# jianwang-mpi/SceneEgo

Hardware: NVIDIA B200
Metric: frames/s VoxelNetDepth volumetric stage (higher is better)
Workload: dtype bf16

## Files before the change

### sceneego_b200/build.py

```python
import concurrent.futures
import hashlib
import os
import subprocess
import sys

HERE = os.path.dirname(os.path.abspath(__file__))
CSRC = os.path.join(HERE, "csrc")
LIB = os.path.join(HERE, "libsceneego_b200.so")
LIB_F16 = os.path.join(HERE, "libsceneego_b200_f16.so")
HASH_FILE = LIB + ".srchash"
OBJ_DIR = os.path.join(HERE, "build")
SOURCES = ["geometry.cu", "softargmax.cu", "v2v.cu", "stem.cu", "stem_march.cu", "tail.cu", "march.cu", "eval.cu", "handoff.cu", "feature_conv.cu"]
NVCC_FLAGS = ["-gencode", "arch=compute_100a,code=sm_100a", "-O3", "-lineinfo", "-std=c++17",
              "-Xcompiler", "-fPIC", "-Xptxas", "-v"]


def _sources():
    return [s for s in SOURCES if os.path.exists(os.path.join(CSRC, s))]


def source_hash() -> str:
    h = hashlib.sha256()
    deps = sorted(os.path.join(CSRC, f) for f in os.listdir(CSRC) if f.endswith((".cu", ".cuh", ".h")))
    deps.append(os.path.join(HERE, "..", "include", "sceneego_b200.h"))
    for d in deps:
        h.update(os.path.basename(d).encode())
        h.update(open(d, "rb").read())
    h.update(" ".join(NVCC_FLAGS + _sources()).encode())
    return h.hexdigest()


def recorded_hash() -> str:
    try:
        return open(HASH_FILE).read().strip()
    except OSError:
        return ""


def _stale() -> bool:
    return not (os.path.exists(LIB) and os.path.exists(LIB_F16)) or recorded_hash() != source_hash()


VARIANTS = [("bf16", LIB, []), ("f16", LIB_F16, ["-DSCENEEGO_ACT_F16"])]


def build(force: bool = False, verbose: bool = False) -> str:
    if not force and not _stale():
        return LIB
    nvcc = os.environ.get("NVCC", "/usr/local/cuda/bin/nvcc")
    os.makedirs(OBJ_DIR, exist_ok=True)
    want = source_hash()

    def compile_one(job):
        tag, src, extra = job
        obj = os.path.join(OBJ_DIR, src.replace(".cu", f".{tag}.o"))
        r = subprocess.run([nvcc] + NVCC_FLAGS + extra + ["-c", os.path.join(CSRC, src), "-o", obj], capture_output=True, text=True)
        return tag, src, obj, r

    jobs = [(tag, src, extra) for tag, _, extra in VARIANTS for src in _sources()]
    jobs.sort(key=lambda j: -os.path.getsize(os.path.join(CSRC, j[1])))
    objs = {tag: [] for tag, _, _ in VARIANTS}
    failed = False
    with concurrent.futures.ThreadPoolExecutor(max_workers=min(8, os.cpu_count() or 1)) as ex:
        for tag, src, obj, r in ex.map(compile_one, jobs):
            if verbose or r.returncode != 0:
                sys.stderr.write(f"---- {src} [{tag}]\n{r.stdout}{r.stderr}")
            failed |= r.returncode != 0
            objs[tag].append(obj)
    if failed:
        raise RuntimeError("nvcc failed building libsceneego_b200")
    for tag, lib, _ in VARIANTS:
        r = subprocess.run([nvcc, "--shared", "-gencode", "arch=compute_100a,code=sm_100a", "-o", lib] + objs[tag],
                           capture_output=True, text=True)
        if verbose or r.returncode != 0:
            sys.stderr.write(r.stdout + r.stderr)
        if r.returncode != 0:
            raise RuntimeError(f"nvcc failed linking {os.path.basename(lib)}")
    with open(HASH_FILE, "w") as f:
        f.write(want + "\n")
    return LIB


if __name__ == "__main__":
    print(build(force="--force" in sys.argv, verbose="-q" not in sys.argv))
```

### sceneego_b200/csrc/common.cuh

```cuda
#pragma once
#include <cuda_runtime.h>
#include <cuda_bf16.h>
#include <cuda_fp16.h>
#include <stdint.h>
#include <stdio.h>
#include "../../include/sceneego_b200.h"

namespace sceneego {

#ifdef SCENEEGO_ACT_F16
constexpr int kActDtype = 1;
constexpr uint32_t kIdescAB = 0u;
#define SE_MMA_SYNC_AB ".f16.f16"
__device__ __forceinline__ uint32_t act_pack2(float lo, float hi) {
  uint32_t r;
  asm("cvt.rn.satfinite.f16x2.f32 %0, %1, %2;" : "=r"(r) : "f"(hi), "f"(lo));
  return r;
}
__device__ __forceinline__ uint32_t act_pack2_relu(float lo, float hi) {
  uint32_t r;
  asm("cvt.rn.relu.satfinite.f16x2.f32 %0, %1, %2;" : "=r"(r) : "f"(hi), "f"(lo));
  return r;
}
__device__ __forceinline__ float2 act_unpack2(uint32_t u) { return __half22float2(*reinterpret_cast<const __half2*>(&u)); }
__device__ __forceinline__ __nv_bfloat16 act_from_float(float v) {
  const uint32_t r = act_pack2(v, 0.f);
  const uint16_t lo = (uint16_t)(r & 0xFFFFu);
  return *reinterpret_cast<const __nv_bfloat16*>(&lo);
}
__device__ __forceinline__ float act_to_float(__nv_bfloat16 v) { return __half2float(*reinterpret_cast<const __half*>(&v)); }
#else
constexpr int kActDtype = 0;
constexpr uint32_t kIdescAB = (1u << 7) | (1u << 10);
#define SE_MMA_SYNC_AB ".bf16.bf16"
__device__ __forceinline__ uint32_t act_pack2(float lo, float hi) {
  const __nv_bfloat162 h = __floats2bfloat162_rn(lo, hi);
  return *reinterpret_cast<const uint32_t*>(&h);
}
__device__ __forceinline__ uint32_t act_pack2_relu(float lo, float hi) {
  uint32_t r;
  asm("cvt.rn.relu.bf16x2.f32 %0, %1, %2;" : "=r"(r) : "f"(hi), "f"(lo));
  return r;
}
__device__ __forceinline__ float2 act_unpack2(uint32_t u) { return __bfloat1622float2(*reinterpret_cast<const __nv_bfloat162*>(&u)); }
__device__ __forceinline__ __nv_bfloat16 act_from_float(float v) { return __float2bfloat16(v); }
__device__ __forceinline__ float act_to_float(__nv_bfloat16 v) { return __bfloat162float(v); }
#endif

void set_error(const char* fmt, ...);
int ensure_max_dynamic_smem(const void* kernel, int bytes);

#define SE_REQUIRE(cond, ...)                      \
  do {                                             \
    if (!(cond)) {                                 \
      ::sceneego::set_error(__VA_ARGS__);          \
      return SCENEEGO_E_INVALID;                   \
    }                                              \
  } while (0)

#define SE_CUDA_LAUNCH_CHECK(what)                                              \
  do {                                                                          \
    cudaError_t e__ = cudaGetLastError();                                       \
    if (e__ != cudaSuccess) {                                                   \
      ::sceneego::set_error("%s: %s", what, cudaGetErrorString(e__));           \
      return SCENEEGO_E_CUDA;                                                   \
    }                                                                           \
  } while (0)

struct CalibDev {
  double cx, cy;
  double c2w[7];
  double w2c[11];
  int width, height;
};

inline CalibDev to_dev(const sceneego_calib_t* c) {
  CalibDev d;
  d.cx = c->cx; d.cy = c->cy;
  for (int i = 0; i < 7; ++i) d.c2w[i] = c->c2w[i];
  for (int i = 0; i < 11; ++i) d.w2c[i] = c->w2c[i];
  d.width = c->width; d.height = c->height;
  return d;
}

__host__ __device__ inline int64_t vol_pos(const sceneego_vol_layout_t& L, int b, int x, int y, int z) {
  return (int64_t)b * L.frame_pitch + L.guard + (int64_t)x * L.pitch_x + (int64_t)y * L.pitch_y + z;
}

__device__ __forceinline__ float voxel_coord(float lo, float step, int i) {
  return __fadd_rn(lo, __fmul_rn(step, (float)i));
}

__host__ __device__ inline int64_t vol_cell(const sceneego_vol_layout_t& L, int b, int x, int y, int z, int g, int C8) {
  if (L.s2d) {
    const int par = ((x & 1) << 2) | ((y & 1) << 1) | (z & 1);
    return (int64_t)(par * C8 + g) * L.plane_stride + vol_pos(L, b, x >> 1, y >> 1, z >> 1);
  }
  return (int64_t)g * L.plane_stride + vol_pos(L, b, x, y, z);
}
__host__ __device__ inline int64_t vol_scene_elem(const sceneego_vol_layout_t& L, int b, int x, int y, int z, int C8) {
  if (L.s2d) {
    const int par = ((x & 1) << 2) | ((y & 1) << 1) | (z & 1);
    return ((int64_t)(8 * C8) * L.plane_stride + vol_pos(L, b, x >> 1, y >> 1, z >> 1)) * 8 + par;
  }
  return ((int64_t)C8 * L.plane_stride + vol_pos(L, b, x, y, z)) * 8;
}

constexpr int kNumSMs = 148;

int launch_stem_s2d(const sceneego_v2v_op_t& op, void* const* d_buffers, const void* d_blob, int batch, int op_index,
                    bool simt, cudaStream_t st);
int launch_feature_conv1x1_simt(const float* d_feat, const float* d_weight, const float* d_bias, float* d_out, int batch,
                                int cin, int cout, int h, int w, cudaStream_t st);
int launch_stem_march(const sceneego_v2v_op_t& op, void* const* d_buffers, const void* d_blob, int batch, int op_index,
                      bool simt, cudaStream_t st);
int launch_tail_mlp(const sceneego_v2v_op_t& op, void* const* d_buffers, const void* d_blob, int batch, int op_index,
                    bool simt, cudaStream_t st);
int launch_conv_march(const sceneego_v2v_op_t& op, void* const* d_buffers, const void* d_blob, int batch, int op_index,
                      cudaStream_t st);

}
```

### sceneego_b200/csrc/v2v.cu

```cuda
#include "tc_common.cuh"
#include <stdarg.h>
#include <stdlib.h>
#include <string.h>
#include <math.h>
#include <mutex>

namespace sceneego {


struct ConvParams {
  const __nv_bfloat16* src;
  __nv_bfloat16* dst;
  const __nv_bfloat16* res;
  float* dst_f32;
  const __nv_bfloat16* w;
  const float* bias;
  sceneego_vol_layout_t ls, ld;
  int batch;
  int k, r, cin_planes, ksteps, N, cout_real, flags;
  int xs, n0, n_dx, n_xg, items_per_plane;
  FastDiv fd_frame, fd_px, fd_py;
  int deconv, par0;
  int taps_dx;
  int mma_n;
// ... 611 lines not shown
  }
  *reinterpret_cast<uint4*>(dst + ((int64_t)g * ld.plane_stride + vol_pos(ld, b, x, y, z)) * 8) = pack8(m);
}

__global__ void __launch_bounds__(128) deconv2_kernel(const __grid_constant__ ConvParams p) {
  const int So = p.ld.side;
  const int n = blockIdx.x * blockDim.x + threadIdx.x;
  const int go = blockIdx.y, b = blockIdx.z;
  if (n >= So * So * So) return;
  const int z = n % So, y = (n / So) % So, x = n / (So * So);
  const int tap = ((x & 1) * 2 + (y & 1)) * 2 + (z & 1);
  const int64_t qs = vol_pos(p.ls, b, x >> 1, y >> 1, z >> 1);
  float acc[8];
#pragma unroll
  for (int j = 0; j < 8; ++j) acc[j] = 0.f;
  for (int g = 0; g < p.cin_planes; ++g) {
    float a[8];
    unpack8(*reinterpret_cast<const uint4*>(p.src + ((int64_t)g * p.ls.plane_stride + qs) * 8), a);
    int npar = 256 / p.N;
    if (npar > 8) npar = 8;
    const uint4* wrow = reinterpret_cast<const uint4*>(p.w) +
                        ((size_t)(tap / npar) * p.cin_planes + g) * ((size_t)npar * p.N) + (size_t)(tap % npar) * p.N + go * 8;
#pragma unroll
    for (int j = 0; j < 8; ++j) {
      float wv[8];
      unpack8(__ldg(wrow + j), wv);
#pragma unroll
      for (int i = 0; i < 8; ++i) acc[j] = fmaf(a[i], wv[i], acc[j]);
    }
  }
  const int64_t cell = (int64_t)go * p.ld.plane_stride + vol_pos(p.ld, b, x, y, z);
  float rr[8];
  if (p.flags & SCENEEGO_F_ADD_AFTER) unpack8(*reinterpret_cast<const uint4*>(p.res + cell * 8), rr);
#pragma unroll
  for (int j = 0; j < 8; ++j) {
    float t = acc[j] + p.bias[go * 8 + j];
    if (p.flags & SCENEEGO_F_RELU) t = fmaxf(t, 0.f);
    if (p.flags & SCENEEGO_F_ADD_AFTER) t += rr[j];
    acc[j] = t;
  }
  *reinterpret_cast<uint4*>(p.dst + cell * 8) = pack8(acc);
}

static thread_local char g_err[512] = "";
int ensure_max_dynamic_smem(const void* kernel, int bytes) {
  struct Entry { int dev; const void* fn; int bytes; };
  static Entry seen[512];
  static int n_seen = 0;
  static std::mutex mu;
  int dev = 0;
  cudaError_t e = cudaGetDevice(&dev);
  if (e != cudaSuccess) { set_error("cudaGetDevice: %s", cudaGetErrorString(e)); return SCENEEGO_E_CUDA; }
  std::lock_guard<std::mutex> lock(mu);
  for (int i = 0; i < n_seen; ++i)
    if (seen[i].dev == dev && seen[i].fn == kernel && seen[i].bytes >= bytes) return SCENEEGO_OK;
  e = cudaFuncSetAttribute(kernel, cudaFuncAttributeMaxDynamicSharedMemorySize, bytes);
  if (e != cudaSuccess) { set_error("cudaFuncSetAttribute(MaxDynamicSharedMemorySize): %s", cudaGetErrorString(e)); return SCENEEGO_E_CUDA; }
  if (n_seen < 512) seen[n_seen++] = Entry{dev, kernel, bytes};
  return SCENEEGO_OK;
}

void set_error(const char* fmt, ...) {
  va_list ap;
  va_start(ap, fmt);
  vsnprintf(g_err, sizeof(g_err), fmt, ap);
  va_end(ap);
}
static thread_local int g_launches = 0;

static bool try_plan(ConvParams& p, int tiles, int want_stages) {
  const int taps_dx = p.taps_dx;
  const int L = tiles * 128;
  const int WL = L + 2 * p.r * (p.ls.pitch_y + 1);
  const uint32_t win_bytes = (uint32_t)WL * 16u;
  const uint32_t stage = win_bytes * p.cin_planes;
  const uint32_t fixed = 1024;
  if ((uint64_t)stage * want_stages + fixed > kMaxSmem) return false;
  const uint32_t used = stage * want_stages + fixed;
  const uint32_t room = kMaxSmem - used;
  int wct = taps_dx, wrows = 0;
  if (p.k == 3 && !p.deconv && 3u * 9u * p.tap_bytes <= room) { wct = 9; wrows = 3; }
  else if (p.k == 3 && !p.deconv && 2u * 3u * p.tap_bytes <= room) { wct = 3; wrows = 1; }
  else {
    while (wct > 1 && (uint32_t)wct * p.tap_bytes > 24576u) {
      int nx = wct - 1;
      while (nx > 1 && taps_dx % nx) --nx;
      wct = nx;
    }
  }
  { const char* e = getenv("SCENEEGO_WCHUNK"); if (e && atoi(e) > 0 && taps_dx % atoi(e) == 0) { wct = atoi(e); wrows = (p.k == 3 && !p.deconv && wct % 3 == 0) ? wct / 3 : 0; if (wrows == 2) wrows = 0; } }
  const uint32_t wchunk = (uint32_t)wct * p.tap_bytes;
  if (2ull * wchunk > room) return false;
  int slots = (int)(room / wchunk);
  if (slots > MAX_WSLOTS) slots = MAX_WSLOTS;
  if (slots > 4 && wchunk > 8192) slots = 4;
  { const char* e = getenv("SCENEEGO_WSLOTS"); if (e && atoi(e) >= 2 && atoi(e) <= MAX_WSLOTS && (uint64_t)used + (uint64_t)atoi(e) * wchunk <= kMaxSmem) slots = atoi(e); }
  p.wrows = wrows;
  p.tiles = tiles; p.L = L; p.WL = WL;
  p.win_bytes = win_bytes; p.win_stages = want_stages;
  p.wchunk_taps = wct; p.wchunks_per_dx = taps_dx / wct; p.wchunk_bytes = wchunk; p.w_slots = slots;
  p.off_win = 0;
  p.off_w = stage * want_stages;
  p.off_bias = p.off_w + wchunk * slots;
  p.off_bar = p.off_bias + 512;
  p.half_cols = (uint32_t)(tiles * p.N);
  uint32_t cols = 32;
  while (cols < 2 * p.half_cols) cols <<= 1;
  p.tmem_cols = cols;
  return true;
}

static int plan_conv(ConvParams& p, int64_t n_pos) {
  p.tap_bytes = (uint32_t)p.cin_planes * (p.mma_n / p.cg) * 16u;
  int max_tiles = 256 / p.N;
  if (max_tiles > 8) max_tiles = 8;
  if (p.xs == 1 && p.cg == 1) {
    auto items_of = [&](int t) { return (n_pos + (int64_t)t * 128 - 1) / ((int64_t)t * 128); };
    if (items_of(max_tiles) < 4 * kNumSMs) {
      int best = max_tiles;
      int64_t best_cost = ((items_of(max_tiles) + kNumSMs - 1) / kNumSMs) * max_tiles;
      for (int t = max_tiles >> 1; t >= 1; t >>= 1) {
        const int64_t cost = ((items_of(t) + kNumSMs - 1) / kNumSMs) * t;
        if (cost < best_cost) { best_cost = cost; best = t; }
      }
      max_tiles = best;
    }
  }
  const char* et = getenv("SCENEEGO_TILES");
  const char* es = getenv("SCENEEGO_STAGES");
  if (et || es) {
    const int tiles = et ? atoi(et) : max_tiles;
    const int stages = es ? atoi(es) : 2;
    if (tiles >= 1 && tiles <= max_tiles && stages >= 1 && stages <= MAX_STAGES && try_plan(p, tiles, stages))
      return (int)(p.off_bar + 512);
  }
  const int first_stages = p.k == 1 ? 4 : (p.cg == 2 || p.cin_planes <= 2) ? 3 : 2;
  for (int tiles = max_tiles; tiles >= 1; tiles >>= 1)
    for (int stages = first_stages; stages >= 2; --stages)
      if (try_plan(p, tiles, stages)) return (int)(p.off_bar + 512);
  return -1;
}

}

using namespace sceneego;

extern "C" int sceneego_abi_version(void) { return SCENEEGO_ABI_VERSION; }
extern "C" int sceneego_act_dtype(void) { return kActDtype; }
extern "C" const char* sceneego_last_error(void) { return g_err; }
extern "C" int sceneego_v2v_last_launch_count(void) { return g_launches; }

extern "C" int sceneego_v2v_pack_conv(const float* h_weight, const float* h_bias, const float* h_gamma,
                                      const float* h_beta, const float* h_mean, const float* h_var, double eps,
                                      int cout, int cin, int ksize, int transposed, int cout_pad, int cin_pad,
                                      int xstack, int n_split, uint16_t* h_w_out, float* h_b_out) {
  SE_REQUIRE(h_weight && h_w_out && h_b_out, "pack_conv: null argument");
  SE_REQUIRE(cout_pad >= cout && cin_pad >= cin && cout_pad % 8 == 0 && cin_pad % 8 == 0, "pack_conv: bad padding");
  SE_REQUIRE(xstack >= 1 && (xstack == 1 || !transposed), "pack_conv: bad xstack");
  SE_REQUIRE(n_split == 1 || (n_split == 2 && !transposed && (xstack * cout_pad) % 32 == 0), "pack_conv: bad n_split");
  const int taps = ksize * ksize * ksize;
  const int kk = ksize * ksize;
  const int n_stk = xstack * cout_pad;
  const int n_dx = ksize + xstack - 1;
  memset(h_w_out, 0, (size_t)n_dx * kk * cin_pad * n_stk * sizeof(uint16_t));
  for (int co = 0; co < cout_pad; ++co) {
    double scale = 1.0, shift = 0.0;
    if (co < cout) {
      if (h_gamma) {
        scale = (double)h_gamma[co] / sqrt((double)h_var[co] + eps);
        shift = (double)h_beta[co] - (double)h_mean[co] * scale;
      }
      h_b_out[co] = (float)((h_bias ? (double)h_bias[co] : 0.0) * scale + shift);
    } else {
      h_b_out[co] = 0.f;
    }
    if (co >= cout) continue;
    for (int ci = 0; ci < cin; ++ci)
      for (int t = 0; t < taps; ++t) {
        const size_t src = transposed ? (((size_t)ci * cout + co) * taps + t) : (((size_t)co * cin + ci) * taps + t);
        const uint16_t wv = f2bf((float)((double)h_weight[src] * scale));
        const int dx = t / kk, rest = t % kk;
        if (transposed) {
          int npar = 256 / cout_pad;
          if (npar > 8) npar = 8;
          const size_t grp = (size_t)t / npar, nrow = (size_t)(t % npar) * cout_pad + co;
          h_w_out[((grp * (cin_pad / 8) + ci / 8) * ((size_t)npar * cout_pad) + nrow) * 8 + (ci & 7)] = wv;
          continue;
        }
        for (int sft = 0; sft < xstack; ++sft) {
          const size_t tp = (size_t)(dx + sft) * kk + rest;
          const size_t col = (size_t)sft * cout_pad + co;
          const size_t nh = (size_t)n_stk / n_split, hf = col / nh;
          const size_t half_elems = (size_t)n_dx * kk * cin_pad * nh;
          const size_t dst = hf * half_elems + ((tp * (cin_pad / 8) + ci / 8) * nh + (col - hf * nh)) * 8 + (ci & 7);
          h_w_out[dst] = wv;
        }
      }
  }
  return SCENEEGO_OK;
}

static int launch_conv_tc(ConvParams& p, int batch, int op_index, cudaStream_t st) {
  p.n0_shift = -1;
  for (int k = 3; k < 10; ++k) if ((1 << k) == p.n0) p.n0_shift = k;
  const int64_t n_pos = (int64_t)batch * p.ls.frame_pitch;
  SE_REQUIRE(n_pos + 4096 < (1ll << 31) && (n_pos + 4096) * (int64_t)p.ls.frame_pitch < (1ll << 48),
             "v2v_run: op %d: batch * frame_pitch too large for one launch (use a smaller chunk)", op_index);
  p.fd_frame = make_fastdiv((uint32_t)p.ls.frame_pitch);
  p.fd_px = make_fastdiv((uint32_t)p.ls.pitch_x);
  p.fd_py = make_fastdiv((uint32_t)p.ls.pitch_y);
  const int smem = plan_conv(p, n_pos);
  SE_REQUIRE(smem > 0, "v2v_run: op %d does not fit shared memory", op_index);
  if (p.xs == 1) {
    p.n_items = (int)((n_pos + p.L - 1) / p.L);
  } else {
    p.items_per_plane = (p.ls.pitch_x + p.L - 1) / p.L;
    p.n_xg = (p.ls.side + p.xs - 1) / p.xs;
    p.n_items = batch * p.n_xg * p.items_per_plane;
  }
  int grid = p.n_items < kNumSMs ? p.n_items : kNumSMs;
  conv_tc_fn fn = nullptr;
  p.w_main_bytes = (uint32_t)(p.n_dx * p.taps_dx) * p.tap_bytes;
  p.w_half_bytes = p.w_main_bytes + (uint32_t)p.n_dx2 * (p.tap_bytes / 2);
  if (p.cg == 2) {
    const int groups = (p.n_items + 1) / 2;
    grid = 2 * (groups < kNumSMs / 2 ? groups : kNumSMs / 2);
    fn = pick_conv_tc_pair(p.ksteps, p.tiles, p.xs, p.wrows);
  } else {
    fn = pick_conv_tc(p.ksteps, p.tiles, p.xs, p.wrows);
    if (fn == nullptr && p.wrows != 0) { p.wrows = 0; fn = pick_conv_tc(p.ksteps, p.tiles, p.xs, 0); }
  }
  SE_REQUIRE(fn != nullptr, "v2v_run: op %d: no conv_tc instantiation for ksteps=%d tiles=%d xs=%d wrows=%d cta_pair=%d", op_index,
             p.ksteps, p.tiles, p.xs, p.wrows, p.cg);
  if (int rc = ensure_max_dynamic_smem((const void*)fn, (int)kMaxSmem)) return rc;
  if (p.cg == 2) {
    cudaLaunchConfig_t cfg;
    memset(&cfg, 0, sizeof(cfg));
    cfg.gridDim = dim3((unsigned)grid); cfg.blockDim = dim3((unsigned)conv_threads(p.tiles));
    cfg.dynamicSmemBytes = (size_t)smem; cfg.stream = st;
    cudaLaunchAttribute attr;
    attr.id = cudaLaunchAttributeClusterDimension;
    attr.val.clusterDim.x = 2; attr.val.clusterDim.y = 1; attr.val.clusterDim.z = 1;
    cfg.attrs = &attr; cfg.numAttrs = 1;
    cudaError_t e = cudaLaunchKernelEx(&cfg, fn, p);
    if (e != cudaSuccess) { set_error("conv_tc (CTA pair): %s", cudaGetErrorString(e)); return SCENEEGO_E_CUDA; }
  } else {
    fn<<<grid, conv_threads(p.tiles), (size_t)smem, st>>>(p);
  }
  SE_CUDA_LAUNCH_CHECK("conv_tc");
  ++g_launches;
  return SCENEEGO_OK;
}

static int v2v_run_impl(const sceneego_v2v_op_t* ops, int n_ops, void* const* d_buffers, const void* d_blob,
                        int batch, void* stream, cudaEvent_t* ev) {
  SE_REQUIRE(ops && d_buffers && d_blob && n_ops > 0 && batch > 0, "v2v_run: bad argument");
  cudaStream_t st = (cudaStream_t)stream;
  const char* force_simt = getenv("SCENEEGO_FORCE_SIMT");
  g_launches = 0;
  for (int i = 0; i < n_ops; ++i) {
    if (ev) cudaEventRecord(ev[i], st);
    const sceneego_v2v_op_t& op = ops[i];
    ConvParams p;
    memset(&p, 0, sizeof(p));
    p.src = (const __nv_bfloat16*)d_buffers[op.src];
    p.dst = (__nv_bfloat16*)d_buffers[op.dst];
    p.dst_f32 = (float*)d_buffers[op.dst];
    p.res = op.res >= 0 ? (const __nv_bfloat16*)d_buffers[op.res] : nullptr;
    p.ls = op.lay_src; p.ld = op.lay_dst; p.batch = batch; p.flags = op.flags;
    SE_REQUIRE(p.src && p.dst, "v2v_run: op %d has a null buffer", i);
    SE_REQUIRE(!(op.flags & (SCENEEGO_F_RESIDUAL | SCENEEGO_F_ADD_AFTER)) || p.res, "v2v_run: op %d needs a residual", i);
    if (op.type == SCENEEGO_OP_MAXPOOL2) {
      SE_REQUIRE(op.lay_dst.side * 2 == op.lay_src.side && op.cin % 8 == 0, "v2v_run: op %d bad pool shape", i);
      const int So = op.lay_dst.side;
      dim3 grid((So * So * So + 255) / 256, op.cin / 8, batch);
      maxpool2_kernel<<<grid, 256, 0, st>>>(p.src, p.dst, p.ls, p.ld, op.cin / 8);
      SE_CUDA_LAUNCH_CHECK("maxpool2");
      ++g_launches;
      continue;
    }
    if (op.type == SCENEEGO_OP_STEM7_S2D || op.type == SCENEEGO_OP_TAIL_MLP || op.type == SCENEEGO_OP_STEM7_MARCH) {
      const bool simt = op.impl == 1 || force_simt;
      const int rc = op.type == SCENEEGO_OP_STEM7_S2D ? launch_stem_s2d(op, d_buffers, d_blob, batch, i, simt, st)
                     : op.type == SCENEEGO_OP_STEM7_MARCH ? launch_stem_march(op, d_buffers, d_blob, batch, i, simt, st)
                                                          : launch_tail_mlp(op, d_buffers, d_blob, batch, i, simt, st);
      if (rc != SCENEEGO_OK) return rc;
      ++g_launches;
      continue;
    }
    p.w = (const __nv_bfloat16*)((const char*)d_blob + op.w_offset);
    p.bias = (const float*)((const char*)d_blob + op.b_offset);
    p.cin_planes = op.cin / 8; p.ksteps = op.cin / 16; p.N = op.cout; p.cout_real = op.cout_real;
    p.xs = 1; p.n0 = op.cout; p.n_dx = op.ksize; p.n_xg = 0; p.items_per_plane = 0; p.cg = 1;
    if (op.type == SCENEEGO_OP_DECONV2) {
      SE_REQUIRE(op.lay_dst.side == 2 * op.lay_src.side && op.cin % 8 == 0 && op.cout % 8 == 0, "v2v_run: op %d bad deconv shape", i);
      if (op.impl == 1 || force_simt || op.cin % 16 || op.cout % 16 || op.cout > 256) {
        const int So = op.lay_dst.side;
        dim3 grid((So * So * So + 127) / 128, op.cout / 8, batch);
        deconv2_kernel<<<grid, 128, 0, st>>>(p);
        SE_CUDA_LAUNCH_CHECK("deconv2");
        ++g_launches;
        continue;
      }
      int npar = 256 / op.cout;
      if (npar > 8) npar = 8;
      const __nv_bfloat16* w_all = p.w;
      for (int par0 = 0; par0 < 8; par0 += npar) {
        ConvParams q = p;
        q.k = 1; q.r = 0; q.xs = 1; q.n0 = op.cout; q.mma_n = npar * op.cout; q.N = npar * op.cout; q.n_dx = 1;
        q.deconv = 1; q.par0 = par0; q.taps_dx = 1;
        q.w = w_all + (size_t)par0 * q.cin_planes * op.cout * 8;
        const int rc = launch_conv_tc(q, batch, i, st);
        if (rc != SCENEEGO_OK) return rc;
      }
      continue;
    }
    if (op.type == SCENEEGO_OP_CONV3_MARCH) {
      if (op.impl == 1 || force_simt) {
        SE_REQUIRE(op.ksize == 3 && op.cin % 16 == 0 && op.cout % 16 == 0, "v2v_run: op %d bad marching conv", i);
        p.k = 3; p.r = 1; p.xs = 1; p.n0 = op.cout; p.N = op.cout; p.cg = 1; p.march = 1;
        p.fd_frame = make_fastdiv((uint32_t)p.ls.frame_pitch);
        p.fd_px = make_fastdiv((uint32_t)p.ls.pitch_x);
        p.fd_py = make_fastdiv((uint32_t)p.ls.pitch_y);
        p.src2 = nullptr; p.n_dx2 = 0;
        if (op.src2 >= 0 && op.cin2 > 0) { p.src2 = (const __nv_bfloat16*)d_buffers[op.src2]; p.n_dx2 = 1; }
        p.w_main_bytes = 27u * (uint32_t)p.cin_planes * (uint32_t)op.cout * 16u;
        p.w_half_bytes = 0;
        const int64_t n_pos = (int64_t)batch * p.ls.frame_pitch;
        dim3 grid((unsigned)((n_pos + 127) / 128), op.cout / 16);
        conv_simt_kernel<<<grid, 128, 0, st>>>(p, n_pos);
        SE_CUDA_LAUNCH_CHECK("conv_simt (march layout)");
      } else {
        const int rc = launch_conv_march(op, d_buffers, d_blob, batch, i, st);
        if (rc != SCENEEGO_OK) return rc;
      }
      ++g_launches;
      continue;
    }
    SE_REQUIRE(op.type == SCENEEGO_OP_CONV, "v2v_run: op %d unknown type", i);
    SE_REQUIRE(op.ksize == 1 || op.ksize == 3 || op.ksize == 7, "v2v_run: op %d unsupported kernel size", i);
    SE_REQUIRE(op.cin % 16 == 0 && op.cout % 16 == 0 && op.cout >= 16 && op.cout <= 128, "v2v_run: op %d channels must be multiples of 16", i);
    SE_REQUIRE(op.lay_src.side == op.lay_dst.side && op.lay_src.pad >= op.ksize / 2 && op.lay_dst.pad <= op.lay_src.pad,
               "v2v_run: op %d layouts incompatible with the stencil", i);
    p.k = op.ksize; p.r = op.ksize / 2;
    const int64_t n_pos = (int64_t)batch * p.ls.frame_pitch;
    p.fd_frame = make_fastdiv((uint32_t)p.ls.frame_pitch);
    p.fd_px = make_fastdiv((uint32_t)p.ls.pitch_x);
    p.fd_py = make_fastdiv((uint32_t)p.ls.pitch_y);
    p.cg = op.cta_pair == 2 ? 2 : 1;
    p.src2 = nullptr; p.n_dx2 = 0;
    if (op.src2 >= 0 && op.cin2 > 0) {
      SE_REQUIRE(op.cin2 * 2 == op.cin && (op.cin / 16) % 2 == 0 && op.ksize == 3 && d_buffers[op.src2],
                 "v2v_run: op %d: a fused shortcut needs a 3^3 conv and a second source with half its channels", i);
      p.src2 = (const __nv_bfloat16*)d_buffers[op.src2];
      p.n_dx2 = op.xstack > 1 ? op.xstack : 1;
    }
    if (op.impl == 1 || force_simt) {
      const int xs_ = op.xstack > 1 ? op.xstack : 1;
      p.n0 = op.cout; p.N = xs_ * op.cout;
      const uint32_t tapb = (uint32_t)p.cin_planes * (p.N / p.cg) * 16u;
      p.w_main_bytes = (uint32_t)((op.ksize + xs_ - 1) * op.ksize * op.ksize) * tapb;
      p.w_half_bytes = p.w_main_bytes + (uint32_t)p.n_dx2 * (tapb / 2);
      dim3 grid((unsigned)((n_pos + 127) / 128), op.cout / 16);
      conv_simt_kernel<<<grid, 128, 0, st>>>(p, n_pos);
      SE_CUDA_LAUNCH_CHECK("conv_simt");
      ++g_launches;
      continue;
    }
    const int xs = op.xstack > 1 ? op.xstack : 1;
    SE_REQUIRE(xs * op.cout <= 256, "v2v_run: op %d: xstack * cout exceeds 256 columns", i);
    SE_REQUIRE(p.cg == 1 || (xs * op.cout) % 32 == 0, "v2v_run: op %d: a CTA pair splits N in halves of whole 16-column groups", i);
    p.xs = xs; p.n0 = op.cout; p.N = xs * op.cout; p.mma_n = p.N; p.n_dx = op.ksize + xs - 1;
    p.deconv = 0; p.par0 = 0; p.taps_dx = op.ksize * op.ksize;
    const int rc = launch_conv_tc(p, batch, i, st);
    if (rc != SCENEEGO_OK) return rc;
  }
  if (ev) cudaEventRecord(ev[n_ops], st);
  return SCENEEGO_OK;
}

extern "C" int sceneego_v2v_run(const sceneego_v2v_op_t* ops, int n_ops, void* const* d_buffers, const void* d_blob,
                                int batch, void* stream) {
  return v2v_run_impl(ops, n_ops, d_buffers, d_blob, batch, stream, nullptr);
}

extern "C" int sceneego_v2v_run_profile(const sceneego_v2v_op_t* ops, int n_ops, void* const* d_buffers,
                                        const void* d_blob, int batch, void* stream, float* h_ms) {
  SE_REQUIRE(h_ms && n_ops > 0 && n_ops < 4096, "v2v_run_profile: bad argument");
  cudaEvent_t* ev = (cudaEvent_t*)malloc(sizeof(cudaEvent_t) * (n_ops + 1));
  for (int i = 0; i <= n_ops; ++i) cudaEventCreate(&ev[i]);
  int rc = v2v_run_impl(ops, n_ops, d_buffers, d_blob, batch, stream, ev);
  if (rc == SCENEEGO_OK) {
    cudaError_t e = cudaEventSynchronize(ev[n_ops]);
    if (e != cudaSuccess) { set_error("v2v_run_profile: %s", cudaGetErrorString(e)); rc = SCENEEGO_E_CUDA; }
    for (int i = 0; i < n_ops && rc == SCENEEGO_OK; ++i) cudaEventElapsedTime(&h_ms[i], ev[i], ev[i + 1]);
  }
  for (int i = 0; i <= n_ops; ++i) cudaEventDestroy(ev[i]);
  free(ev);
  return rc;
}
```

Before: 3077.

## Add warp-specialized persistent tcgen05 deconv kernel with TMA bulk stores

Adds a dedicated persistent transposed-conv (deconv2) kernel. It uses warp specialization: a loader warp issues bulk async copies, an MMA warp drives tcgen05 into double-buffered TMEM, epilogue warps stage outputs in shared memory, and a store warp writes them out with bulk copies. It covers all 8 output parities in one launch with resident weights, replacing multiple per-parity generic conv launches. This is meant to cut launch count, overlap load, compute and store, and keep weights on chip. In exchange it adds a complex mbarrier pipeline that only some shapes can use.

```diff
diff --git a/sceneego_b200/build.py b/sceneego_b200/build.py
--- a/sceneego_b200/build.py
+++ b/sceneego_b200/build.py
@@ -10,7 +10,7 @@
 LIB_F16 = os.path.join(HERE, "libsceneego_b200_f16.so")
 HASH_FILE = LIB + ".srchash"
 OBJ_DIR = os.path.join(HERE, "build")
-SOURCES = ["geometry.cu", "softargmax.cu", "v2v.cu", "stem.cu", "stem_march.cu", "tail.cu", "march.cu", "eval.cu", "handoff.cu", "feature_conv.cu"]
+SOURCES = ["geometry.cu", "softargmax.cu", "v2v.cu", "stem.cu", "stem_march.cu", "tail.cu", "march.cu", "deconv.cu", "eval.cu", "handoff.cu", "feature_conv.cu"]
 NVCC_FLAGS = ["-gencode", "arch=compute_100a,code=sm_100a", "-O3", "-lineinfo", "-std=c++17",
               "-Xcompiler", "-fPIC", "-Xptxas", "-v"]
 
diff --git a/sceneego_b200/csrc/common.cuh b/sceneego_b200/csrc/common.cuh
--- a/sceneego_b200/csrc/common.cuh
+++ b/sceneego_b200/csrc/common.cuh
@@ -118,5 +118,8 @@
                     bool simt, cudaStream_t st);
 int launch_conv_march(const sceneego_v2v_op_t& op, void* const* d_buffers, const void* d_blob, int batch, int op_index,
                       cudaStream_t st);
+bool deconv_tc_supports(const sceneego_v2v_op_t& op);
+int launch_deconv_tc(const sceneego_v2v_op_t& op, void* const* d_buffers, const void* d_blob, int batch, int op_index,
+                     cudaStream_t st);
 
 }
diff --git a/sceneego_b200/csrc/deconv.cu b/sceneego_b200/csrc/deconv.cu
--- /dev/null
+++ b/sceneego_b200/csrc/deconv.cu
@@ -0,0 +1,331 @@
+#include "tc_common.cuh"
+#include <stdlib.h>
+#include <string.h>
+
+namespace sceneego {
+
+constexpr int DC_ROWS = 128;
+constexpr int DC_FIRST_EPI = 3;
+constexpr int DC_EPI_WARPS = 8;
+constexpr int DC_THREADS = 32 * (DC_FIRST_EPI + DC_EPI_WARPS);
+constexpr uint32_t DC_TMEM_COLS = 512;
+
+struct DeconvParams {
+  const __nv_bfloat16* src;
+  const __nv_bfloat16* res;
+  __nv_bfloat16* dst;
+  const uint8_t* w;
+  const float* bias;
+  sceneego_vol_layout_t ls, ld;
+  int batch, flags, ksteps, cin_planes, cout, cout_shift, npar, n_groups, N, n_items;
+  int gpu, upar, n_units, nbuf;
+  int lines, items_per_plane;
+  int w_resident, win_stages;
+  uint32_t win_bytes, group_bytes, run_bytes, img_bytes;
+  uint32_t off_w, off_win, off_bias, off_bar;
+};
+
+__device__ __forceinline__ void bulk_s2g(void* dst, uint32_t src, uint32_t bytes) {
+  asm volatile("cp.async.bulk.global.shared::cta.bulk_group [%0], [%1], %2;" ::"l"(dst), "r"(src), "r"(bytes) : "memory");
+}
+__device__ __forceinline__ void bulk_commit() { asm volatile("cp.async.bulk.commit_group;" ::: "memory"); }
+__device__ __forceinline__ void bulk_wait_read_all() { asm volatile("cp.async.bulk.wait_group.read 0;" ::: "memory"); }
+__device__ __forceinline__ void bulk_wait_all() { asm volatile("cp.async.bulk.wait_group 0;" ::: "memory"); }
+
+struct DcItem {
+  int64_t q0;
+  int64_t dbase;
+  int nl;
+};
+__device__ __forceinline__ DcItem dc_item(const DeconvParams& p, int item) {
+  const int yi = item % p.items_per_plane, t = item / p.items_per_plane;
+  const int x = t % p.ls.side, b = t / p.ls.side, y0 = yi * p.lines;
+  DcItem d;
+  d.q0 = (int64_t)b * p.ls.frame_pitch + p.ls.guard + (int64_t)x * p.ls.pitch_x + (int64_t)y0 * p.ls.pitch_y;
+  d.dbase = (int64_t)b * p.ld.frame_pitch + p.ld.guard + (int64_t)(2 * x) * p.ld.pitch_x + (int64_t)(2 * y0) * p.ld.pitch_y;
+  d.nl = min(p.lines, p.ls.side - y0);
+  return d;
+}
+
+template <class G>
+__device__ __forceinline__ void for_each_copy(const DeconvParams& p, const DcItem& d, int u, int lane, G&& g) {
+  const int planes = p.cout >> 3, npx = p.upar >> 2;
+  const uint32_t bytes = (uint32_t)(2 * d.nl * p.ld.pitch_y) * 16u;
+  for (int ci = lane; ci < npx * planes; ci += 32) {
+    const int j = ci / planes, c8 = ci - j * planes;
+    const int px = ((u * p.upar) >> 2) + j;
+    g((uint32_t)ci * p.run_bytes, (int64_t)c8 * p.ld.plane_stride + d.dbase + (int64_t)px * p.ld.pitch_x, bytes);
+  }
+}
+
+__global__ void __launch_bounds__(DC_THREADS, 1) deconv2_tc_kernel(const __grid_constant__ DeconvParams p) {
+  extern __shared__ __align__(128) uint8_t smem[];
+  const int warp = __shfl_sync(0xffffffffu, (int)(threadIdx.x >> 5), 0);
+  const int lane = threadIdx.x & 31;
+  const uint32_t sbase = smem_u32(smem);
+  float* s_bias = reinterpret_cast<float*>(smem + p.off_bias);
+  const uint32_t bar0 = sbase + p.off_bar;
+  auto BAR = [&](int i) { return bar0 + 8u * (uint32_t)i; };
+  constexpr int B_WIN_FULL = 0, B_WIN_EMPTY = 2, B_W_FULL = 4, B_W_EMPTY = 5, B_TM_FULL = 6, B_TM_EMPTY = 8,
+                B_IMG_FULL = 10, B_IMG_DONE = 12, B_IMG_FREE = 14, B_COUNT = 16;
+  uint32_t* s_tmem_ptr = reinterpret_cast<uint32_t*>(smem + p.off_bar + 8 * B_COUNT);
+
+  for (int i = threadIdx.x; i < p.cout; i += DC_THREADS) s_bias[i] = p.bias[i];
+  if (threadIdx.x == 0) {
+    for (int i = 0; i < 2; ++i) {
+      mbar_init(BAR(B_WIN_FULL + i), 1); mbar_init(BAR(B_WIN_EMPTY + i), 1);
+      mbar_init(BAR(B_TM_FULL + i), 1); mbar_init(BAR(B_TM_EMPTY + i), DC_EPI_WARPS);
+      mbar_init(BAR(B_IMG_FULL + i), 32); mbar_init(BAR(B_IMG_DONE + i), DC_EPI_WARPS); mbar_init(BAR(B_IMG_FREE + i), 1);
+    }
+    mbar_init(BAR(B_W_FULL), 1); mbar_init(BAR(B_W_EMPTY), 1);
+    asm volatile("fence.mbarrier_init.release.cluster;" ::: "memory");
+  }
+  if (warp == 1) {
+    asm volatile("tcgen05.alloc.cta_group::1.sync.aligned.shared::cta.b32 [%0], %1;" ::"r"(smem_u32(s_tmem_ptr)), "r"(DC_TMEM_COLS)
+                 : "memory");
+    asm volatile("tcgen05.relinquish_alloc_permit.cta_group::1.sync.aligned;" ::: "memory");
+  }
+  tc_fence_before();
+  __syncthreads();
+  tc_fence_after();
+  const uint32_t tmem_base = *s_tmem_ptr;
+  const int my_items = (p.n_items - (int)blockIdx.x + (int)gridDim.x - 1) / (int)gridDim.x;
+  const int ng = p.n_groups;
+  auto item_of = [&](int it) { return dc_item(p, (int)blockIdx.x + it * (int)gridDim.x); };
+  const bool skip = (p.flags & (SCENEEGO_F_ADD_AFTER | SCENEEGO_F_RESIDUAL)) != 0;
+
+  if (warp == 0) {
+    auto copy_w = [&](int gi, uint32_t dst) {
+      for (uint32_t o = 0; o < p.group_bytes; o += 16384u)
+        bulk_g2s(dst + o, p.w + (size_t)gi * p.group_bytes + o, min(p.group_bytes - o, 16384u), BAR(B_W_FULL));
+    };
+    if (p.w_resident && lane == 0) {
+      mbar_expect_tx(BAR(B_W_FULL), (uint32_t)ng * p.group_bytes);
+      for (int gi = 0; gi < ng; ++gi) copy_w(gi, sbase + p.off_w + (uint32_t)gi * p.group_bytes);
+    }
+    int k = 0, kw = 0;
+    for (int it = 0; it < my_items; ++it) {
+      const DcItem d = item_of(it);
+      const int ws = it % p.win_stages, wph = (it / p.win_stages) & 1;
+      if (lane == 0) {
+        mbar_wait(BAR(B_WIN_EMPTY + ws), wph ^ 1);
+        mbar_expect_tx(BAR(B_WIN_FULL + ws), p.win_bytes);
+        for (int g = 0; g < p.cin_planes; ++g)
+          bulk_g2s(sbase + p.off_win + (uint32_t)ws * p.win_bytes + (uint32_t)g * (DC_ROWS * 16), p.src + ((int64_t)g * p.ls.plane_stride + d.q0) * 8,
+                   DC_ROWS * 16, BAR(B_WIN_FULL + ws));
+      }
+      for (int u = 0; u < p.n_units; ++u, ++k) {
+        const int buf = k & 1;
+        mbar_wait(BAR(B_IMG_FREE + buf), ((k >> 1) & 1) ^ 1);
+        const uint32_t img = sbase + (uint32_t)buf * p.img_bytes;
+        uint32_t bytes = 0;
+        if (skip) for_each_copy(p, d, u, lane, [&](uint32_t, int64_t, uint32_t n) { bytes += n; });
+        mbar_expect_tx(BAR(B_IMG_FULL + buf), bytes);
+        if (skip)
+          for_each_copy(p, d, u, lane, [&](uint32_t so, int64_t cell, uint32_t n) {
+            bulk_g2s(img + so, p.res + cell * 8, n, BAR(B_IMG_FULL + buf));
+          });
+        if (!p.w_resident && lane == 0) {
+          for (int h = 0; h < p.gpu; ++h, ++kw) {
+            mbar_wait(BAR(B_W_EMPTY), (kw & 1) ^ 1);
+            mbar_expect_tx(BAR(B_W_FULL), p.group_bytes);
+            copy_w(u * p.gpu + h, sbase + p.off_w);
+          }
+        }
+      }
+    }
+  } else if (warp == 1) {
+    const uint32_t tmem_u = __shfl_sync(0xffffffffu, tmem_base, 0);
+    const bool leader = elect_one();
+    const uint32_t idesc = (1u << 4) | kIdescAB | ((uint32_t)(p.N >> 3) << 17) | (8u << 24);
+    const uint64_t desc_hi = (uint64_t)(8u | (1u << 14)) << 32;
+    const uint32_t a_lo_flags = (uint32_t)(DC_ROWS * 16 >> 4) << 16;
+    const uint32_t b_lo_flags = (((uint32_t)p.N * 16u >> 4) & 0x3FFFu) << 16;
+    const uint32_t a_ks_step = 2u * DC_ROWS * 16u >> 4, b_ks_step = 2u * (uint32_t)p.N * 16u >> 4;
+    int k = 0, kw = 0;
+    for (int it = 0; it < my_items; ++it) {
+      const int ws = it % p.win_stages, wph = (it / p.win_stages) & 1;
+      mbar_wait_warp(BAR(B_WIN_FULL + ws), wph);
+      const uint32_t a_lo = (((sbase + p.off_win + (uint32_t)ws * p.win_bytes) >> 4) & 0x3FFFu) | a_lo_flags;
+      for (int u = 0; u < p.n_units; ++u, ++k) {
+        const int abuf = p.nbuf == 2 ? (k & 1) : 0, aph = p.nbuf == 2 ? ((k >> 1) & 1) : (k & 1);
+        mbar_wait_warp(BAR(B_TM_EMPTY + abuf), aph ^ 1);
+        for (int h = 0; h < p.gpu; ++h) {
+          const int gi = u * p.gpu + h;
+          mbar_wait_warp(BAR(B_W_FULL), p.w_resident ? 0 : (kw & 1));
+          tc_fence_after();
+          const uint32_t w_addr = sbase + p.off_w + (p.w_resident ? (uint32_t)gi * p.group_bytes : 0u);
+          const uint32_t b_lo = ((w_addr >> 4) & 0x3FFFu) | b_lo_flags;
+          if (leader) {
+            for (int ks = 0; ks < p.ksteps; ++ks)
+              tc_mma_bf16(tmem_u + (uint32_t)abuf * 256u + (uint32_t)(h * p.N), desc_hi | (a_lo + (uint32_t)ks * a_ks_step),
+                          desc_hi | (b_lo + (uint32_t)ks * b_ks_step), idesc, ks == 0 ? 0u : 1u);
+            if (!p.w_resident) tc_commit(BAR(B_W_EMPTY));
+          }
+          if (!p.w_resident) ++kw;
+          __syncwarp();
+        }
+        if (leader) {
+          if (u == p.n_units - 1) tc_commit(BAR(B_WIN_EMPTY + ws));
+          tc_commit(BAR(B_TM_FULL + abuf));
+        }
+        __syncwarp();
+      }
+    }
+  } else if (warp == 2) {
+    int k = 0;
+    for (int it = 0; it < my_items; ++it) {
+      const DcItem d = item_of(it);
+      for (int u = 0; u < p.n_units; ++u, ++k) {
+        const int buf = k & 1;
+        mbar_wait(BAR(B_IMG_DONE + buf), (k >> 1) & 1);
+        const uint32_t img = sbase + (uint32_t)buf * p.img_bytes;
+        for_each_copy(p, d, u, lane, [&](uint32_t so, int64_t cell, uint32_t n) { bulk_s2g(p.dst + cell * 8, img + so, n); });
+        bulk_commit();
+        bulk_wait_read_all();
+        __syncwarp();
+        if (lane == 0) mbar_arrive(BAR(B_IMG_FREE + buf));
+      }
+    }
+    bulk_wait_all();
+  } else {
+    const int quarter = warp & 3;
+    const int half = (warp - DC_FIRST_EPI) >> 2;
+    const int row = quarter * 32 + lane;
+    const int nch = (p.gpu * p.N) >> 4, planes = p.cout >> 3, S = p.ls.side, Pd = p.ld.pitch_y;
+    const int l = row / p.ls.pitch_y, z = row - l * p.ls.pitch_y;
+    const uint32_t taddr0 = tmem_base + ((uint32_t)(quarter * 32) << 16);
+    int k = 0;
+    for (int it = 0; it < my_items; ++it) {
+      const bool line_ok = l < item_of(it).nl && z <= S;
+      for (int u = 0; u < p.n_units; ++u, ++k) {
+        const int buf = k & 1;
+        const int abuf = p.nbuf == 2 ? (k & 1) : 0, aph = p.nbuf == 2 ? ((k >> 1) & 1) : (k & 1);
+        uint8_t* img = smem + (size_t)buf * p.img_bytes;
+        mbar_wait(BAR(B_TM_FULL + abuf), aph);
+        mbar_wait(BAR(B_IMG_FULL + buf), (k >> 1) & 1);
+        tc_fence_after();
+#pragma unroll 1
+        for (int c = half; c < nch; c += 2) {
+          uint32_t raw[16];
+          tc_ld16(taddr0 + (uint32_t)abuf * 256u + (uint32_t)(c << 4), raw);
+          const int pl = (c << 4) >> p.cout_shift;
+          const int ch0 = (c << 4) - (pl << p.cout_shift);
+          tc_wait_ld();
+          float bs[16];
+#pragma unroll
+          for (int j = 0; j < 4; ++j) {
+            const float4 b4 = *reinterpret_cast<const float4*>(s_bias + ch0 + 4 * j);
+            bs[4 * j] = b4.x; bs[4 * j + 1] = b4.y; bs[4 * j + 2] = b4.z; bs[4 * j + 3] = b4.w;
+          }
+          const int pz = pl & 1;
+          const bool active = line_ok && !(z == S && pz);
+#pragma unroll
+          for (int g = 0; g < 2; ++g) {
+            if (!active) break;
+            uint4* cellp = reinterpret_cast<uint4*>(img) +
+                           ((((pl >> 2) * planes + (ch0 >> 3) + g) * 2 * p.lines + 2 * l + ((pl >> 1) & 1)) * Pd + 2 * z + pz);
+            if (z == S) { *cellp = make_uint4(0, 0, 0, 0); continue; }
+            float rr[8];
+            if (skip) unpack8(*cellp, rr);
+            float o[8];
+#pragma unroll
+            for (int j = 0; j < 8; ++j) {
+              float t = __uint_as_float(raw[8 * g + j]) + bs[8 * g + j];
+              if (p.flags & SCENEEGO_F_RESIDUAL) t += rr[j];
+              if (p.flags & SCENEEGO_F_RELU) t = fmaxf(t, 0.f);
+              if (p.flags & SCENEEGO_F_ADD_AFTER) t += rr[j];
+              o[j] = t;
+            }
+            *cellp = pack8(o);
+          }
+        }
+        tc_fence_before();
+        asm volatile("fence.proxy.async.shared::cta;" ::: "memory");
+        __syncwarp();
+        if (lane == 0) {
+          mbar_arrive(BAR(B_TM_EMPTY + abuf));
+          mbar_arrive(BAR(B_IMG_DONE + buf));
+        }
+      }
+    }
+  }
+  tc_fence_before();
+  __syncthreads();
+  if (warp == 1) asm volatile("tcgen05.dealloc.cta_group::1.sync.aligned.b32 %0, %1;" ::"r"(tmem_base), "r"(DC_TMEM_COLS) : "memory");
+}
+
+static uint32_t deconv_plan(const sceneego_v2v_op_t& op, DeconvParams& p) {
+  p.ls = op.lay_src; p.ld = op.lay_dst; p.flags = op.flags;
+  const int S = p.ls.side;
+  p.cin_planes = op.cin / 8;
+  p.ksteps = op.cin / 16;
+  p.cout = op.cout;
+  for (p.cout_shift = 4; (1 << p.cout_shift) < op.cout; ++p.cout_shift) {}
+  p.npar = 256 / op.cout > 8 ? 8 : 256 / op.cout;
+  p.n_groups = 8 / p.npar;
+  p.N = p.npar * op.cout;
+  p.gpu = p.npar >= 4 ? 1 : 2;
+  p.upar = p.npar * p.gpu;
+  p.n_units = 8 / p.upar;
+  p.nbuf = p.gpu == 1 ? 2 : 1;
+  p.win_bytes = (uint32_t)p.cin_planes * DC_ROWS * 16u;
+  p.group_bytes = (uint32_t)p.cin_planes * (uint32_t)p.N * 16u;
+  const uint32_t fixed = 512u + 256u;
+  for (int max_lines = min(DC_ROWS / p.ls.pitch_y, S); max_lines >= 1; --max_lines) {
+    p.items_per_plane = (S + max_lines - 1) / max_lines;
+    p.lines = (S + p.items_per_plane - 1) / p.items_per_plane;
+    p.run_bytes = (uint32_t)(2 * p.lines * p.ld.pitch_y) * 16u;
+    p.img_bytes = ((uint32_t)(p.upar / 4) * (uint32_t)(op.cout / 8) * p.run_bytes + 1023u) / 1024u * 1024u;
+    const uint64_t imgs = 2ull * p.img_bytes;
+    if (imgs + (uint64_t)p.n_groups * p.group_bytes + 2ull * p.win_bytes + fixed <= kMaxSmem) {
+      p.w_resident = 1; p.win_stages = 2;
+    } else {
+      p.w_resident = 0;
+      p.win_stages = imgs + p.group_bytes + 2ull * p.win_bytes + fixed <= kMaxSmem ? 2 : 1;
+    }
+    p.off_w = (uint32_t)imgs;
+    p.off_win = p.off_w + (p.w_resident ? (uint32_t)p.n_groups : 1u) * p.group_bytes;
+    p.off_bias = p.off_win + (uint32_t)p.win_stages * p.win_bytes;
+    p.off_bar = p.off_bias + 512u;
+    if (p.off_bar + 256u <= kMaxSmem) return p.off_bar + 256u;
+  }
+  return 0;
+}
+
+bool deconv_tc_supports(const sceneego_v2v_op_t& op) {
+  if (!(op.cin % 16 == 0 && op.cin <= 256 && (op.cout == 16 || op.cout == 32 || op.cout == 64 || op.cout == 128) &&
+        !(op.flags & SCENEEGO_F_OUT_F32) && op.lay_src.s2d == 0 && op.lay_dst.s2d == 0 && op.lay_src.zwin == 0 &&
+        op.lay_dst.zwin == 0 && op.lay_src.pad >= 1 && op.lay_dst.pad == 1 && op.lay_src.pitch_y <= DC_ROWS &&
+        op.lay_dst.side == 2 * op.lay_src.side))
+    return false;
+  DeconvParams p;
+  memset(&p, 0, sizeof(p));
+  if (deconv_plan(op, p) == 0) return false;
+  return p.gpu == 1 || p.items_per_plane == 1;
+}
+
+int launch_deconv_tc(const sceneego_v2v_op_t& op, void* const* d_buffers, const void* d_blob, int batch, int op_index,
+                     cudaStream_t st) {
+  SE_REQUIRE(deconv_tc_supports(op), "v2v_run: op %d: shape not supported by deconv2_tc_kernel", op_index);
+  DeconvParams p;
+  memset(&p, 0, sizeof(p));
+  const uint32_t smem = deconv_plan(op, p);
+  p.src = (const __nv_bfloat16*)d_buffers[op.src];
+  p.dst = (__nv_bfloat16*)d_buffers[op.dst];
+  p.res = op.res >= 0 ? (const __nv_bfloat16*)d_buffers[op.res] : nullptr;
+  p.w = (const uint8_t*)d_blob + op.w_offset;
+  p.bias = (const float*)((const char*)d_blob + op.b_offset);
+  p.batch = batch;
+  SE_REQUIRE(!(op.flags & (SCENEEGO_F_ADD_AFTER | SCENEEGO_F_RESIDUAL)) || p.res, "v2v_run: op %d needs a skip tensor", op_index);
+  const int S = p.ls.side;
+  SE_REQUIRE((int64_t)batch * S * p.items_per_plane < (1ll << 31), "v2v_run: op %d: too many work items for one launch", op_index);
+  p.n_items = batch * S * p.items_per_plane;
+  const int grid = p.n_items < kNumSMs ? p.n_items : kNumSMs;
+  if (int rc = ensure_max_dynamic_smem((const void*)deconv2_tc_kernel, (int)kMaxSmem)) return rc;
+  deconv2_tc_kernel<<<grid, DC_THREADS, smem, st>>>(p);
+  SE_CUDA_LAUNCH_CHECK("deconv2_tc");
+  return SCENEEGO_OK;
+}
+
+}
diff --git a/sceneego_b200/csrc/v2v.cu b/sceneego_b200/csrc/v2v.cu
--- a/sceneego_b200/csrc/v2v.cu
+++ b/sceneego_b200/csrc/v2v.cu
@@ -937,6 +937,13 @@
         ++g_launches;
         continue;
       }
+      const char* generic = getenv("SCENEEGO_DECONV_GENERIC");
+      if (!(generic && atoi(generic) == 1) && deconv_tc_supports(op)) {
+        const int rc = launch_deconv_tc(op, d_buffers, d_blob, batch, i, st);
+        if (rc != SCENEEGO_OK) return rc;
+        ++g_launches;
+        continue;
+      }
       int npar = 256 / op.cout;
       if (npar > 8) npar = 8;
       const __nv_bfloat16* w_all = p.w;
```

Measured after the change: 3124 (median of 6 runs). +1.5%, better.
